# alessioGalatolo/GAN-2D-to-3D

Measured on AMD Instinct MI355X. Metric: GAN2Shape step iters/sec, faces 128×128 b=8, 1/2/4/8 MI355X, higher is better.
Workload: dtype f32; 1 GPU; face128_n8; image_size=128, gan_size=128, n_proj_samples=8, mfma_operands=f32, prior=ellipsoid, step_mix=7:7:6 (step1:step2:step3, main.py:148 stage 0), images_per_rank=1

## Files before the change

### gan-2d-to-3d_amd/csrc/modconv.hip

```cpp
#include "modconv_desc.h"
#include "conv_wgrad_core.h"
#include "thinconv.h"
#include "xcd_tile.h"

namespace g2s {

template <int T> struct KTile {
    static constexpr int BKT = (T == 9) ? 18 : (T == 25) ? 26 : 16;
    static constexpr int CPT = BKT / T;
    static constexpr int KMAX = (T == 25) ? 26 : 18;
};

template <int BM, int BN, int T, bool PARTIAL, bool SCALE>
__device__ __forceinline__ void modconv_body(const ConvDesc &d, const ConvClass &c,
                                             float (&As)[2][KTile<T>::KMAX][BM + 1],
                                             float (&Bs)[2][KTile<T>::KMAX + 1][BN],
                                             const int (&stab)[25], const int tile_id, const int grp,
                                             const int kt_begin, const int kt_end, const bool atomic) {
    constexpr int BKT = KTile<T>::BKT, CPT = KTile<T>::CPT, BK_MAX = KTile<T>::KMAX;
    constexpr int WAVES_M = BM >= 64 ? 2 : 1, WAVES_N = 4 / WAVES_M;
    constexpr int WMT = BM / (32 * WAVES_M), WNT = BN / (32 * WAVES_N);
    constexpr bool WIDE = (T == 9);
    constexpr int EA = WIDE ? (BM * 6 + NTHREADS - 1) / NTHREADS : (BM * BKT + NTHREADS - 1) / NTHREADS;
    constexpr int EB = (BN * BKT + NTHREADS - 1) / NTHREADS;
    const int tid = threadIdx.x, lane = tid & 63, wave = tid >> 6;
    const int wm = wave / WAVES_N, wn = wave % WAVES_N;
    const int Ncls = d.B * c.OH * c.OW;
    const int tiles_m = (d.M + BM - 1) / BM;
    const int m0 = (tile_id % tiles_m) * BM;
    const int n0 = (tile_id / tiles_m) * BN;
    const int HW = d.H * d.W;
    constexpr int OOB = 0x7fffffff;

    const auto rx = __builtin_amdgcn_make_buffer_rsrc((void *)(d.x + (size_t)grp * d.Cr * HW), 0,
                                                      (d.B * d.Cx - grp * d.Cr) * HW * 4, 0x00020000);
    const auto rw = __builtin_amdgcn_make_buffer_rsrc((void *)(d.w + (size_t)grp * (d.w_bytes / 4)), 0, d.w_bytes, 0x00020000);
    const auto rsc = __builtin_amdgcn_make_buffer_rsrc(
        (void *)(SCALE ? d.in_scale : d.w), 0, SCALE ? d.B * d.Cr * 4 : 4, 0x00020000);

    const int nB = tid % BN;
    const int ng = n0 + nB;
    const bool n_ok = ng < Ncls;
    int bb = 0, iy0 = 0, ix0 = 0;
    if (n_ok) {
        bb = ng / (c.OH * c.OW);
        const int r = ng % (c.OH * c.OW);
        iy0 = (r / c.OW) * d.is;
        ix0 = (r % c.OW) * d.is;
    }
    int offB[EB], dchB[EB];
#pragma unroll
// ... 121 lines not shown
                for (int j = 0; j < WNT; j++) {
                    acc[i][j] = __builtin_amdgcn_mfma_f32_32x32x2f32(a[p][i], b[p][j], acc[i][j], 0, 0, 0);
                    if (slot == 0 && st < EA) storeA(st, anext);
                    if (slot == (WMT * WNT > 1 ? 1 : 0) && st < EA) loadA(st, kt2);
                    if (slot == (WMT * WNT > 2 ? 2 : 0) && st < EB) storeB(st, bnext);
                    if (slot == (WMT * WNT > 3 ? 3 : 0) && st < EB) loadB(st, kt2);
                    slot++;
                }
            __builtin_amdgcn_sched_group_barrier(0x100, WMT + WNT, 0);
            for (int q = 0; q < WMT * WNT; q++) {
                __builtin_amdgcn_sched_group_barrier(0x008, 1, 0);
                __builtin_amdgcn_sched_group_barrier(0x200, 1, 0);
                __builtin_amdgcn_sched_group_barrier(0x020, 2, 0);
                __builtin_amdgcn_sched_group_barrier(0x002, 4, 0);
            }
        }
        if constexpr (WIDE && SCALE) { rs[0] = rsn[0]; rs[1] = rsn[1]; }
        asm volatile("s_waitcnt lgkmcnt(0)\n\ts_barrier" ::: "memory");
    };
    int kt = kt_begin;
    for (; kt + 1 < kt_end; kt += 2) {
        ktile(kt, 0);
        ktile(kt + 1, 1);
    }
    if (kt < kt_end) ktile(kt, 0);

#pragma unroll
    for (int j = 0; j < WNT; j++) {
        const int n = n0 + wn * (BN / WAVES_N) + j * 32 + l31;
        if (n >= Ncls) continue;
        const int b = n / (c.OH * c.OW);
        const int r_ = n % (c.OH * c.OW);
        const int oy = (r_ / c.OW) * d.os + c.oy0, ox = (r_ % c.OW) * d.os + c.ox0;
        float *yb = d.y + (((size_t)b * d.My + grp * d.M) * d.OHf + oy) * d.OWf + ox;
        const float *ob = d.out_scale ? d.out_scale + (size_t)b * d.M : nullptr;
        const float *gbias = d.bias ? d.bias + grp * d.M : nullptr;
        const float nz = d.noise ? d.noise_w[0] * d.noise[oy * d.OWf + ox] : 0.0f;
#pragma unroll
        for (int i = 0; i < WMT; i++)
#pragma unroll
            for (int r = 0; r < 16; r++) {
                const int m = m0 + wm * (BM / WAVES_M) + i * 32 + (r & 3) + 8 * (r >> 2) + 4 * lk;
                if (m >= d.M) continue;
                float v = acc[i][j][r];
                if (ob) v *= ob[m];
                if (gbias) v += gbias[m];
                v += nz;
                if (d.act) v = (v > 0.0f ? v : v * d.act_alpha) * d.act_gain;
                float *dst = yb + (size_t)m * d.OHf * d.OWf;
                if (atomic) unsafeAtomicAdd(dst, v);
                else *dst = v;
            }
    }
}

static __host__ __device__ inline int ktiles_of(int Cr, int T) {
    const int cpt = (T == 9) ? 2 : (T == 25) ? 1 : 16 / T;
    return (Cr + cpt - 1) / cpt;
}

template <int BM, int BN, int KMAX>
__device__ __forceinline__ void modconv_segment(const ConvDesc &d, const ConvClass &c,
                                                float (&As)[2][KMAX][BM + 1], float (&Bs)[2][KMAX + 1][BN],
                                                const int (&stab)[25], const int tile_id, const int grp,
                                                const int kb, const int ke, const bool atomic) {
    const bool scale = d.in_scale != nullptr;
#define G2S_BODY(T, PART, SC) modconv_body<BM, BN, T, PART, SC>(d, c, As, Bs, stab, tile_id, grp, kb, ke, atomic)
#define G2S_TAPS(T, CPT)                                   \
    if (d.Cr % CPT) {                                      \
        if (scale) G2S_BODY(T, true, true);                \
        else G2S_BODY(T, true, false);                     \
    } else {                                               \
        if (scale) G2S_BODY(T, false, true);               \
        else G2S_BODY(T, false, false);                    \
    }
    if constexpr (KMAX == 26) {
        G2S_BODY(25, true, false);
    } else {
        switch (c.T) {
        case 9: G2S_TAPS(9, 2) break;
        case 16: G2S_BODY(16, true, false); break;
        case 4: G2S_TAPS(4, 4) break;
        case 2: G2S_TAPS(2, 8) break;
        default: G2S_TAPS(1, 16) break;
        }
    }
#undef G2S_TAPS
#undef G2S_BODY
}

template <int BM, int BN, int KMAX>
__device__ __forceinline__ void modconv_block(const ConvDesc &d, float (&As)[2][KMAX][BM + 1],
                                              float (&Bs)[2][KMAX + 1][BN], int (&stab)[25], const int nx,
                                              const int bx, const int by, const int bz, const int row) {
    const int tiles_m = (d.M + BM - 1) / BM;
    const int tile_all0 = __builtin_amdgcn_readfirstlane(xcd_logical_tile(nx, bx, row));
    const ConvClass &c = d.cls[bz];
    const int mt_all = tile_all0 % (tiles_m * d.groups);
    const int grp = __builtin_amdgcn_readfirstlane(mt_all / tiles_m);
    const int tile_id = __builtin_amdgcn_readfirstlane((tile_all0 / (tiles_m * d.groups)) * tiles_m + mt_all % tiles_m);
    if ((int)(tile_id / tiles_m) * BN >= d.B * c.OH * c.OW) return;
    const int ktiles = ktiles_of(d.Cr, c.T);
    const int slices = d.cls_splitk[bz];
    const int per = (ktiles + slices - 1) / slices;
    const int kb = by * per;
    if (by >= slices || kb >= ktiles) return;
    if (threadIdx.x < 25) stab[threadIdx.x] = c.tab[threadIdx.x];
    __syncthreads();
    modconv_segment<BM, BN, KMAX>(d, c, As, Bs, stab, tile_id, grp, kb, min(ktiles, kb + per), slices > 1);
}

template <int BM, int BN, int KMAX>
__global__ __launch_bounds__(NTHREADS) void modconv_kernel(ConvDesc d) {
    __shared__ float As[2][KMAX][BM + 1];
    __shared__ float Bs[2][KMAX + 1][BN];
    __shared__ int stab[25];
    modconv_block<BM, BN, KMAX>(d, As, Bs, stab, gridDim.x, blockIdx.x, blockIdx.y, blockIdx.z,
                                blockIdx.y + gridDim.y * blockIdx.z);
}

__global__ __launch_bounds__(NTHREADS) void conv_wgrad_rider_kernel(WgradParams p) {
    __shared__ float Wa[WG_BK][WG_BM + 1];
    __shared__ float Wb[WG_BK][WG_BN + 1];
    wgrad_block(p, Wa, Wb, blockIdx.x, blockIdx.y, blockIdx.z);
}

template <int BM, int BN, int KMAX>
__global__ __launch_bounds__(NTHREADS) void conv_bwd_kernel(ConvDesc d, WgradParams p, int nx, int ny, int n_dgrad,
                                                            int w_tiles, int w_split) {
    __shared__ float As[2][KMAX][BM + 1];
    __shared__ float Bs[2][KMAX + 1][BN];
    __shared__ int stab[25];
    __shared__ float Wa[WG_BK][WG_BM + 1];
    __shared__ float Wb[WG_BK][WG_BN + 1];
    const int lin = blockIdx.x;
    if (lin < n_dgrad) {
        const int bx = lin % nx, row = lin / nx;
        modconv_block<BM, BN, KMAX>(d, As, Bs, stab, nx, bx, row % ny, row / ny, row);
    } else {
        const int l = lin - n_dgrad;
        const int bx = l % w_tiles, r = l / w_tiles;
        wgrad_block(p, Wa, Wb, bx, r % w_split, r / w_split);
    }
}

}

using namespace g2s;

struct TunedConv { int B, Cin, Cout, H, k, mode, transpose, fused, tile, splitk; };
static const TunedConv kTuned[] = {
#include "modconv_tuned.inc"
    {0, 0, 0, 0, 0, 0, 0, 0, 0, 0}};
// ... 21 lines not shown

struct WgradRider {
    WgradParams p;
    int tiles, split;
    bool dw_is_zero;
};

struct Epilogue {
    const float *bias, *noise, *noise_w;
    int act;
    float alpha, gain;
};

template <int KMAX>
static void conv_launch_tile(const ConvDesc &d, const dim3 grid, const int pick, hipStream_t st,
                             const WgradRider *rider = nullptr) {
    const int n_dgrad = grid.x * grid.y * grid.z;
#define G2S_TILE(BM_, BN_)                                                                                           \
    if (rider)                                                                                                       \
        conv_bwd_kernel<BM_, BN_, KMAX><<<n_dgrad + rider->tiles * rider->split * rider->p.groups, NTHREADS, 0, st>>>( \
            d, rider->p, grid.x, grid.y, n_dgrad, rider->tiles, rider->split);                                       \
    else                                                                                                             \
        modconv_kernel<BM_, BN_, KMAX><<<grid, NTHREADS, 0, st>>>(d)
    switch (pick) {
    case 0: modconv_kernel<128, 128, KMAX><<<grid, NTHREADS, 0, st>>>(d); break;
    case 1: modconv_kernel<128, 64, KMAX><<<grid, NTHREADS, 0, st>>>(d); break;
    case 2: G2S_TILE(64, 64); break;
    case 3: G2S_TILE(32, 128); break;
    default: G2S_TILE(64, 128); break;
    }
#undef G2S_TILE
}

static int conv_launch(const float *x, const float *w, const float *in_scale, const float *out_scale,
                       const Epilogue &ep, float *y, int B, int Cr, int M, int H, int W, const ConvGeom &g,
                       int tuned_tile, int tuned_splitk, g2s_stream_t stream, bool y_is_zero = false,
                       bool f16_operands = false, int groups = 1, const WgradRider *rider = nullptr,
                       int *plan_needs_zero = nullptr) {
    G2S_REQUIRE(plan_needs_zero || (x && w && y), "x, w, y must not be NULL");
    G2S_REQUIRE(B > 0 && Cr > 0 && M > 0 && H > 0 && W > 0, "sizes must be positive");
    const int k = g.k, s_ = g.stride, p_ = g.pad, KK = k * k;
    G2S_REQUIRE(k >= 1 && k <= 5, "kernel size must be 1..5 (got %d)", k);
    G2S_REQUIRE(s_ == 1 || s_ == 2, "stride must be 1 or 2 (got %d)", s_);
    G2S_REQUIRE(p_ >= 0 && p_ < k, "padding must be in [0, k)");
    ConvDesc d{};
    d.x = x;
    d.w = w;
    d.in_scale = in_scale;
    d.out_scale = out_scale;
    d.bias = ep.bias;
    d.noise = ep.noise;
    d.noise_w = ep.noise_w;
    G2S_REQUIRE(!d.noise || (!f16_operands && groups == 1), "the noise epilogue exists for the fp32 kernel only");
    d.act = ep.act;
    d.act_alpha = ep.alpha;
    d.act_gain = ep.gain;
    d.y = y;
    d.B = B;
    d.H = H;
    d.W = W;
    d.Cr = Cr;
    d.M = M;
    d.w_ms = g.m_major ? Cr * KK : KK;
    d.w_ks = g.m_major ? KK : M * KK;
    d.w_bytes = M * Cr * KK * 4;
    G2S_REQUIRE(groups >= 1 && groups <= 8 && (groups == 1 || (!in_scale && !out_scale && !f16_operands)),
                "grouped launches take no input / output scales and fp32 operands");
    d.groups = groups;
    d.Cx = groups * Cr;
    d.My = groups * M;
    bool holes = false;
    if (!g.adjoint) {
// ... 26 lines not shown
                c.ox0 = rx;
                c.OH = (d.OHf - ry + s_ - 1) / s_;
                c.OW = (d.OWf - rx + s_ - 1) / s_;
                c.T = 0;
                for (int ky = 0; ky < k; ky++)
                    for (int kx = 0; kx < k; kx++)
                        if ((ry + p_ - ky) % s_ == 0 && (rx + p_ - kx) % s_ == 0)
                            c.tab[c.T++] = pack((ry + p_ - ky) / s_, (rx + p_ - kx) / s_, ky * k + kx);
                if (c.T == 0 || c.OH <= 0 || c.OW <= 0) {
                    holes = holes || (c.OH > 0 && c.OW > 0);
                    continue;
                }
                d.cls[d.ncls++] = c;
            }
        G2S_REQUIRE(d.ncls > 0, "empty convolution");
    }
    bool big = false;
    for (int i = 0; i < d.ncls; i++) {
        const int T = d.cls[i].T;
        G2S_REQUIRE(T == 1 || T == 2 || T == 4 || T == 9 || T == 16 || T == 25,
                    "unsupported tap count %d (k=%d stride=%d)", T, k, s_);
        G2S_REQUIRE(!(in_scale && T > 9), "input scales are limited to kernels of up to 3x3");
        big = big || T == 25;
    }
    long nmax = 0;
    int kt_min = 1 << 30;
    for (int i = 0; i < d.ncls; i++) {
        nmax = std::max(nmax, (long)B * d.cls[i].OH * d.cls[i].OW);
        kt_min = std::min(kt_min, ktiles_of(d.Cr, d.cls[i].T));
    }
    G2S_REQUIRE(nmax < (1l << 30) && (long)B * d.Cx * H * W < (1l << 29) && (long)groups * M * Cr * KK < (1l << 29),
                "problem too large for 32-bit byte offsets");
    hipStream_t st = as_stream(stream);
    const int cfgs[5][2] = {{128, 128}, {128, 64}, {64, 64}, {32, 128}, {64, 128}};
    int pick = 2;
    for (int i = 0; i < 3; i++) {
        const long blocks = (long)groups * cdiv(d.M, cfgs[i][0]) * cdiv(nmax, cfgs[i][1]) * d.ncls;
        if (d.M > cfgs[i][0] / 2 && blocks >= 512) { pick = i; break; }
    }
    if (d.M <= 32 && nmax >= 1024 && !f16_operands) pick = 3;
    if (f16_operands && pick == 1) pick = 2;
    if (tuned_tile >= 0 && g_force_tile != -2) pick = tuned_tile;
    else tuned_splitk = -1;
    if (g_force_tile >= 0) pick = g_force_tile;
    const int BMv = cfgs[pick][0], BNv = cfgs[pick][1];
    const int tiles = groups * cdiv(d.M, BMv) * cdiv(nmax, BNv);
    int splitk = 1;
    while ((long)tiles * d.ncls * splitk < 512 && kt_min / (splitk * 2) >= 8 && splitk < 64) splitk *= 2;
    if (tuned_splitk > 0) splitk = tuned_splitk;
    if (g_force_splitk > 0) splitk = g_force_splitk;
    if (deterministic()) splitk = 1;
    splitk = std::max(1, std::min(splitk, kt_min));
    dim3 grid(tiles, splitk, d.ncls);
    const bool split = splitk > 1;
    const bool deferred_epilogue = (split || holes) && (ep.bias != nullptr || ep.act != 0 || ep.noise != nullptr);
    if (deferred_epilogue) {
        d.bias = nullptr;
        d.noise = d.noise_w = nullptr;
        d.act = 0;
    }
    d.splitk = splitk;
    int kt_max = 1;
    for (int i = 0; i < d.ncls; i++) kt_max = std::max(kt_max, ktiles_of(d.Cr, d.cls[i].T));
    for (int i = 0; i < d.ncls; i++) {
        const int kt = ktiles_of(d.Cr, d.cls[i].T);
        d.cls_splitk[i] = std::max(1, std::min(kt, (int)(((long)splitk * kt + kt_max / 2) / kt_max)));
// ... 7 lines not shown
            return fail(G2S_ERR_LAUNCH, "hipMemsetAsync(y) failed");
    }
    if (f16_operands) {
        const int rc = modconv_f16_launch(d, grid, pick, st);
        if (rc != G2S_OK) return rc;
    } else if (rider) {
        const WgradParams &p = rider->p;
        if (p.atomic && !rider->dw_is_zero &&
            hipMemsetAsync(p.dw, 0, (size_t)p.groups * p.Ca * p.N * sizeof(float), st) != hipSuccess)
            return fail(G2S_ERR_LAUNCH, "hipMemsetAsync(dw) failed");
        if (big) conv_launch_tile<26>(d, grid, pick, st, pick >= 2 ? rider : nullptr);
        else conv_launch_tile<18>(d, grid, pick, st, pick >= 2 ? rider : nullptr);
        if (pick < 2) conv_wgrad_rider_kernel<<<dim3(rider->tiles, rider->split, p.groups), NTHREADS, 0, st>>>(p);
    } else if (big) {
        conv_launch_tile<26>(d, grid, pick, st);
    } else {
        conv_launch_tile<18>(d, grid, pick, st);
    }
    int rc = check_launch("g2s_modconv");
    if (rc != G2S_OK || !deferred_epilogue) return rc;
    if (ep.noise) {
        G2S_REQUIRE(ep.bias && ep.act == 1, "noise epilogue: needs a bias and act = 1");
        return g2s_noise_bias_act(y, ep.noise, ep.noise_w, ep.bias, y, B, d.My, d.OHf * d.OWf, ep.alpha, ep.gain,
                                  stream);
    }
    return g2s_fused_bias_act(y, ep.bias, nullptr, y, (int64_t)B * d.My * d.OHf * d.OWf,
                              (int64_t)d.OHf * d.OWf, d.My, ep.act ? 3 : 1, 0, ep.alpha,
                              ep.act ? ep.gain : 1.0f, G2S_F32, stream);
}

static int modconv_launch(const float *x, const float *w, const float *in_scale,
                          const float *out_scale, const Epilogue &ep, float *y, int B, int Cin, int Cout, int H,
                          int W, int k, int mode, int transpose, g2s_stream_t stream, bool f16_operands = false,
                          bool y_is_zero = false, int *plan_needs_zero = nullptr) {
    G2S_REQUIRE(B > 0 && Cin > 0 && Cout > 0 && H > 0 && W > 0, "sizes must be positive");
    G2S_REQUIRE(k == 1 || k == 3, "kernel size must be 1 or 3 (got %d)", k);
    G2S_REQUIRE(mode == G2S_CONV_PLAIN || mode == G2S_CONV_UP2 || mode == G2S_CONV_DOWN2,
                "unsupported mode %d", mode);
    if (!f16_operands && !in_scale && !out_scale && !ep.noise && mode == G2S_CONV_PLAIN && g_force_tile == -1 &&
        g_force_splitk == -1 && thin_conv_eligible(B, Cin, Cout, H, W, k, transpose)) {
        if (plan_needs_zero) {
            *plan_needs_zero = 0;
            return G2S_OK;
        }
        return thin_conv_launch(x, w, ep.bias, y, B, Cin, Cout, H, W, ep.act, ep.alpha, ep.gain, stream);
    }
    ConvGeom g{};
    g.k = k;
    g.stride = mode == G2S_CONV_PLAIN ? 1 : 2;
    g.pad = mode == G2S_CONV_PLAIN ? k / 2 : 0;
    g.adjoint = (mode == G2S_CONV_UP2) != (transpose != 0);
    g.m_major = !transpose;
    if (!g.adjoint && mode != G2S_CONV_PLAIN) G2S_REQUIRE(H >= k && W >= k, "input smaller than the kernel");
    int tile = -1, splitk = -1;
    if (H == W && !f16_operands)
        for (int pass = 0; pass < 2 && tile == -1 && splitk == -1; pass++)
            for (const TunedConv *t = kTuned; t->B; ++t)
                if (t->B == B && t->Cin == Cin && t->Cout == Cout && t->H == H && t->k == k && t->mode == mode &&
                    t->transpose == transpose && (pass == 1 || t->fused == (ep.bias != nullptr || ep.act != 0))) {
                    tile = t->tile;
                    splitk = t->splitk;
                    break;
                }
    return conv_launch(x, w, in_scale, out_scale, ep, y, B, transpose ? Cout : Cin, transpose ? Cin : Cout, H, W, g,
                       tile, splitk, stream, y_is_zero, f16_operands, 1, nullptr, plan_needs_zero);
}

extern "C" int g2s_modconv(const float *x, const float *w, const float *in_scale, const float *out_scale,
                           const float *bias, const float *noise, const float *noise_w, float *y, int B, int Cin,
                           int Cout, int H, int W, int k, int mode, int transpose, int act, float alpha, float gain,
                           int y_is_zero, g2s_stream_t stream) {
    G2S_REQUIRE(act == 0 || act == 1, "act must be 0 (none) or 1 (leaky-ReLU)");
    G2S_REQUIRE(!noise || (bias && noise_w && act == 1), "a noise needs bias, noise_w and act = 1");
    return modconv_launch(x, w, in_scale, out_scale, Epilogue{bias, noise, noise_w, act, alpha, gain}, y, B, Cin,
                          Cout, H, W, k, mode, transpose, stream, false, y_is_zero != 0);
}

extern "C" int g2s_modconv_needs_zero(int B, int Cin, int Cout, int H, int W, int k, int mode, int transpose,
                                      int has_scales, int fused) {
    int needs = 0;
    static const float dummy = 0.0f;
    const float *sc = has_scales ? &dummy : nullptr;
    const Epilogue ep{fused ? &dummy : nullptr, nullptr, nullptr, fused ? 1 : 0, 0.0f, 1.0f};
    const int rc = modconv_launch(nullptr, nullptr, sc, nullptr, ep, nullptr, B, Cin, Cout, H, W, k, mode, transpose,
                                  nullptr, false, false, &needs);
    return rc == G2S_OK ? needs : rc;
}

extern "C" int g2s_modconv_f16(const float *x, const float *w, const float *in_scale, const float *out_scale,
                               const float *bias, float *y, int B, int Cin, int Cout, int H, int W, int k,
                               int mode, int transpose, int act, float alpha, float gain, g2s_stream_t stream) {
    G2S_REQUIRE(act == 0 || act == 1, "act must be 0 (none) or 1 (leaky-ReLU)");
    return modconv_launch(x, w, in_scale, out_scale, Epilogue{bias, nullptr, nullptr, act, alpha, gain}, y, B, Cin,
                          Cout, H, W, k, mode, transpose, stream, true);
}

static int conv2d_impl(const float *x, const float *w, const float *bias, float *y, int B, int Cr, int M, int H,
                       int W, int k, int stride, int pad, int adjoint, int w_m_major, int out_h, int out_w,
                       int act, float alpha, float gain, int y_is_zero, int groups, g2s_stream_t stream,
                       const WgradRider *rider = nullptr) {
    G2S_REQUIRE(act == 0 || act == 1, "act must be 0 (none) or 1 (leaky-ReLU)");
    ConvGeom g{k, stride, pad, adjoint ? 1 : 0, w_m_major ? 1 : 0, adjoint ? out_h : 0, adjoint ? out_w : 0};
    int tile = -1, splitk = -1;
    if (H == W)
        for (const TunedConv2d *t = kTuned2d; t->B; ++t)
            if (t->B == B && t->Cr == Cr && t->M == M && t->H == H && t->k == k && t->stride == stride &&
                t->pad == pad && t->adjoint == g.adjoint && t->m_major == g.m_major &&
                t->fused == (bias != nullptr || act != 0) && t->groups == groups) {
// ... 28 lines not shown
```

### gan-2d-to-3d_amd/lib.py

```python
import ctypes as C
import os

import torch

_HERE = os.path.dirname(os.path.abspath(__file__))
LIB_PATH = os.path.join(_HERE, "lib", "libg2s.so")

G2S_F32, G2S_F16 = 0, 1
CONV_PLAIN, CONV_UP2, CONV_DOWN2 = 0, 1, 2

_lib = None

_p, _i, _f, _sz, _i64, _d = C.c_void_p, C.c_int, C.c_float, C.c_size_t, C.c_int64, C.c_double
SIGNATURES = {
    "g2s_abi_version": (_i, []),
    "g2s_last_error": (C.c_char_p, []),
    "g2s_clamp": (_i, [_p, _p, _p, _i64, _f, _f, _i, _p]),
    "g2s_avg_pyramid": (_i, [_p, _p, _i, _i64, _i, _i, _p]),
    "g2s_res_split_fwd": (_i, [_p, _p, _p, _i64, _i, _i, _p]),
    "g2s_res_split_bwd": (_i, [_p, _p, _p, _p, _i64, _i, _i, _p]),
    "g2s_depth_head_fwd": (_i, [_p, _p, _p, _i64, _i, _f, _f, _i, _f, _p]),
    "g2s_depth_head_bwd": (_i, [_p, _p, _p, _p, _p, _i64, _i, _f, _f, _i, _f, _i, _p]),
    "g2s_grid_sample_fwd": (_i, [_p, _p, _p, _i, _i, _i, _i, _i, _i, _i, _f, _f, _p]),
    "g2s_grid_sample_bwd_workspace_bytes": (_sz, [_i, _i, _i, _i]),
# ... 1 lines not shown
    "g2s_set_deterministic": (_i, [_i]),
    "g2s_get_deterministic": (_i, []),
    "g2s_raster_workspace_bytes": (_sz, [_i, _i, _i, _i]),
    "g2s_raster_tune": (_i, [_i]),
    "g2s_raster_get_tune": (_i, []),
    "g2s_raster_depth_fwd": (_i, [_p, _p, _i, _i, _i, _i, _p, _f, _i, _i, _f, _f, _p, _p, _p, _p, _sz, _p]),
    "g2s_raster_depth_bwd": (_i, [_p, _p, _p, _p, _p, _i, _i, _i, _i, _p, _f, _i, _p, _p]),
    "g2s_raster_bwd_workspace_bytes": (_sz, [_i, _i]),
    "g2s_raster_depth_bwd_ex": (_i, [_p, _p, _p, _p, _p, _i, _i, _i, _i, _p, _f, _i, _p, _p, _sz, _i, _p]),
    "g2s_raster_rgb_fwd": (_i, [_p, _p, _p, _p, _p, _i, _i, _i, _i, _i, _i, _i, _p, _f, _p, _p]),
    "g2s_raster_rgb_bwd_workspace_bytes": (_sz, [_i, _i, _i, _i, _i]),
    "g2s_raster_rgb_bwd": (_i, [_p] * 6 + [_i, _i, _i, _i, _p, _f, _i, _i, _i, _f, _p, _p, _p, _sz, _i, _p]),
    "g2s_face_light_fwd": (_i, [_p, _p, _i, _i, _i, _i, _i, _p, _p, _p, _p, _p]),
    "g2s_face_light_bwd": (_i, [_p, _p, _p, _i, _i, _i, _i, _i, _p, _p, _p, _p, _sz, _i, _p]),
    "g2s_raster_rgba_fwd": (_i, [_p] * 6 + [_i, _i, _i, _i, _i, _i, _i, _i, _p, _f, _p, _p, _p]),
    "g2s_raster_rgba_bwd_workspace_bytes": (_sz, [_i, _i, _i, _i, _i, _i]),
    "g2s_raster_rgba_bwd": (_i, [_p] * 7 + [_i, _i, _i, _i, _p, _f, _i, _i, _i, _i, _f, _p, _p, _p, _p, _sz, _i, _p]),
    "g2s_sweep_verts": (_i, [_p, _p, _p, _i, _i, _i, _p]),
    "g2s_sweep_shade": (_i, [_p] * 8 + [_i] * 9 + [_p, _f, _p, _p, _p]),
    "g2s_sweep_pseudo": (_i, [_p] * 8 + [_f, _f, _i, _i, _i, _i, _p, _p, _p]),
    "g2s_mapping_tile": (_i, []),
    "g2s_mapping_fwd": (_i, [_p, _p, _p, _p, _p, _p, _i64, _i, _i, _i, _f, _f, _f, _p]),
    "g2s_rows_mean": (_i, [_p, _p, _i64, _i, _i64, _p]),
    "g2s_image_to_u8": (_i, [_p, _p, _i64, _i, _i, _p]),
    "g2s_fused_bias_act": (_i, [_p, _p, _p, _p, _i64, _i64, _i64, _i, _i, _f, _f, _i, _p]),
    "g2s_maxpool2x2_fwd": (_i, [_p, _p, _i64, _i, _i, _p]),
    "g2s_maxpool2x2_bwd": (_i, [_p, _p, _p, _i64, _i, _i, _p]),
    "g2s_add_bias_scale": (_i, [_p, _p, _p, _p, _i64, _i64, _i, _f, _p]),
    "g2s_noise_bias_act": (_i, [_p, _p, _p, _p, _p, _i, _i, _i, _f, _f, _p]),
    "g2s_noise_bias_act_ps": (_i, [_p, _p, _p, _p, _p, _i, _i, _i, _f, _f, _p]),
    "g2s_upfirdn2d": (_i, [_p, _p, _p] + [_i] * 14 + [_p]),
    "g2s_modconv": (_i, [_p] * 8 + [_i] * 9 + [_f, _f, _i, _p]),
    "g2s_modconv_needs_zero": (_i, [_i, _i, _i, _i, _i, _i, _i, _i, _i, _i]),
    "g2s_upfirdn2d_nba": (_i, [_p, _p, _p] + [_i] * 12 + [_p, _p, _p, _f, _f, _p]),
    "g2s_synth_bwd_rows": (_i, [_p] * 13 + [_i, _i, _i, _f, _f, _p]),
    "g2s_upfirdn2d_nba_ps": (_i, [_p, _p, _p] + [_i] * 12 + [_p, _p, _p, _f, _f, _p]),
    "g2s_synth_bwd_rows_ps": (_i, [_p] * 13 + [_i, _i, _i, _f, _f, _p]),
    "g2s_channel_sum": (_i, [_p, _p, _i, _i, _i, _p]),
    "g2s_noise_grad": (_i, [_p, _p, _p, _i, _i, _i, _p]),
    "g2s_noise_regularize_workspace_bytes": (_sz, [_p, _i, _i]),
    "g2s_noise_regularize": (_i, [_p, _p, _p, _i, _i, _p, _p, _sz, _p]),
    "g2s_noise_normalize_workspace_bytes": (_sz, [_p, _i, _i]),
    "g2s_noise_normalize": (_i, [_p, _p, _i, _i, _p, _sz, _p]),
    "g2s_demod_fwd_multi": (_i, [_p, _p, _p, _p, _p, _i, _i, _f, _p]),
    "g2s_demod_bwd_multi": (_i, [_p, _p, _p, _p, _p, _p, _p, _i, _i, _p]),
    "g2s_modconv_f16": (_i, [_p, _p, _p, _p, _p, _p, _i, _i, _i, _i, _i, _i, _i, _i, _i, _f, _f, _p]),
    "g2s_modconv_tune": (_i, [_i, _i]),
    "g2s_mfma_probe": (_i, [_p, _i, _i, _i, _p]),
    "g2s_mfma_lds_probe": (_i, [_p, _i, _i, _i, _i, _p]),
    "g2s_wino_weights_floats": (_sz, [_i, _i]),
    "g2s_wino4_weights_floats": (_sz, [_i, _i]),
    "g2s_wino4_weights": (_i, [_p, _p, _i, _i, _i, _p]),
    "g2s_wino4_supported": (_i, [_i] * 5),
    "g2s_conv3x3_wino4": (_i, [_p] * 8 + [_i] * 6 + [_f, _f, _i, _p, _i64, _p]),
    "g2s_wino_weights": (_i, [_p, _p, _i, _i, _i, _p]),
    "g2s_conv3x3_wino": (_i, [_p] * 8 + [_i] * 6 + [_f, _f, _i, _p, _i64, _p]),
    "g2s_conv2d": (_i, [_p, _p, _p, _p] + [_i] * 12 + [_i, _f, _f, _i, _i, _p]),
    "g2s_conv2d_wgrad": (_i, [_p, _p, _p] + [_i] * 10 + [_i, _i, _p]),
    "g2s_conv2d_bwd": (_i, [_p, _p, _p] + [_i] * 13 + [_p, _p, _p] + [_i] * 8 + [_p]),
    "g2s_adam_chunk": (_i64, []),
    "g2s_adam_step": (_i, [_p, _p, _p, _i, _i, _f, _f, _f, _f, _f, _p]),
    "g2s_rows_dot_scale": (_i, [_p, _p, _p, _p, _p, _p, _i, _i, _p]),
    "g2s_demod_fwd": (_i, [_p, _p, _p, _i, _i, _i, _f, _p]),
    "g2s_demod_bwd": (_i, [_p, _p, _p, _p, _p, _i, _i, _i, _p]),
    "g2s_demod_bwd_add": (_i, [_p, _p, _p, _p, _p, _p, _i, _i, _i, _p]),
    "g2s_lpips_layer_fwd": (_i, [_p, _p, _p, _p, _i, _i, _i, _p]),
# ... 124 lines not shown
```

### gan-2d-to-3d_amd/modconv.py

```python
import os

import torch
from torch.autograd import Function

from . import lib as _lib
from . import zeropool as _zp

PLAIN, UP2, DOWN2 = _lib.CONV_PLAIN, _lib.CONV_UP2, _lib.CONV_DOWN2

PROFILE = None


class profiled:

    def __init__(self, flop, nbytes, mfma_flop=None, kernel=None):
        self.rec = PROFILE
        self.flop, self.nbytes = flop, nbytes
        self.kernel = kernel or ("direct" if mfma_flop is None else "winograd")
        self.mfma_flop = flop if mfma_flop is None else mfma_flop

    def __enter__(self):
        if self.rec is not None:
            self.e0 = torch.cuda.Event(enable_timing=True)
            self.e1 = torch.cuda.Event(enable_timing=True)
# ... 51 lines not shown
    if tiles < WINO_MIN_TILES or blocks * -(-Cr // 4) < 256 * 32 or M <= 32:
        return None
    return 0


WINO4 = os.environ.get("G2S_WINO4", "1") != "0"


def wino4_supported(B, Cr, M, H, W):
    return WINO4 and _lib.load().g2s_wino4_supported(B, Cr, M, H, W) == 1


_WINO_U = {"winograd": {}, "winograd4": {}}


def _wino_weights(w, transpose, kernel):
    cache = _WINO_U[kernel]
    key = (w.data_ptr(), w._version, tuple(w.shape), int(transpose))
    hit = cache.get(key)
    if hit is None:
        if len(cache) > 256:
            cache.clear()
        Cout, Cin = w.shape[:2]
        L = _lib.load()
        M, Cr = (Cin, Cout) if transpose else (Cout, Cin)
        floats, transform = ((L.g2s_wino4_weights_floats, L.g2s_wino4_weights) if kernel == "winograd4"
                             else (L.g2s_wino_weights_floats, L.g2s_wino_weights))
        U = torch.empty(floats(M, Cr), dtype=torch.float32, device=w.device)
        _lib.check(transform(_lib.ptr(w), _lib.ptr(U), Cout, Cin, int(transpose), _lib.stream()))
        hit = cache[key] = (w, U)
    return hit[1]


def _conv(x, w, in_scale, out_scale, mode, transpose, out_shape, route, bias=None, noise=None, noise_w=None, act=0,
          alpha=0.0, gain=1.0):
    B, Cr, H, W = x.shape
    Cout, Cin, k, _ = w.shape
    M = out_shape[1]
    act, alpha, gain = int(act), float(alpha), float(gain)
    L = _lib.load()
    p = _lib.ptr
    y = None
    if route is None and L.g2s_modconv_needs_zero(B, Cin, Cout, H, W, k, mode, int(transpose),
                                                  int(in_scale is not None or out_scale is not None),
                                                  int(bias is not None or act != 0)) == 1:
        y = _zp.take(out_shape, x.device)
    zeroed = y is not None
    if y is None:
        y = torch.empty(out_shape, dtype=torch.float32, device=x.device)
    oh, ow = out_shape[2], out_shape[3]
    flop = 2.0 * B * Cout * Cin * k * k * (oh * ow if mode == PLAIN else min(H * W, oh * ow))
    nbytes = 4.0 * (x.numel() + w.numel() + y.numel())
    if route is None:
        with profiled(flop, nbytes):
            _lib.check(L.g2s_modconv(p(x), p(w), p(in_scale), p(out_scale), p(bias), p(noise), p(noise_w), p(y), B,
                                     Cin, Cout, H, W, k, mode, int(transpose), act, alpha, gain, int(zeroed),
                                     _lib.stream()))
    elif route == "f16":
        with profiled(flop, nbytes):
            _lib.check(L.g2s_modconv_f16(p(x), p(w), p(in_scale), p(out_scale), p(bias), p(y), B, Cin, Cout, H, W, k,
                                         mode, int(transpose), act, alpha, gain, _lib.stream()))
    elif isinstance(route, str):
        U = _wino_weights(w, transpose, "winograd4")
        with profiled(flop, nbytes, 2.0 * 36 * B * (H // 4) * (W // 4) * M * Cr, "winograd4"):
            _lib.check(L.g2s_conv3x3_wino4(p(x), p(U), p(in_scale), p(out_scale), p(bias), p(noise), p(noise_w), p(y),
                                           B, Cr, M, H, W, act, alpha, gain, int(route[3:] or 0), *_lib.split_ws(),
                                           _lib.stream()))
    else:
        U = _wino_weights(w, transpose, "winograd")
        tiles = B * ((H + 1) // 2) * ((W + 1) // 2)
        with profiled(flop, nbytes, 2.0 * 16 * tiles * M * Cr):
            _lib.check(L.g2s_conv3x3_wino(p(x), p(U), p(in_scale), p(out_scale), p(bias), p(noise), p(noise_w), p(y),
                                          B, Cr, M, H, W, act, alpha, gain, int(route), *_lib.split_ws(),
                                          _lib.stream()))
    return y


def modconv_nba_raw(x, w, in_scale, out_scale, bias, noise, noise_w, slope, gain):
    _lib.require_cuda(x, w, in_scale, out_scale, bias, noise, noise_w)
    if OPERANDS != "f32" or x.dtype != torch.float32:
        raise RuntimeError("modconv_nba: fp32 kernels only")
    x, w = x.contiguous(), w.contiguous()
    B, C, H, W = x.shape
    Cout, Cin = w.shape[:2]
    if C != Cin or tuple(noise.shape[-2:]) != (H, W) or noise.numel() != H * W:
        raise RuntimeError("modconv_nba: shape mismatch")
    si, so = in_scale.contiguous(), out_scale.contiguous()
    bias, noise, noise_w = bias.contiguous(), noise.contiguous(), noise_w.contiguous()
    return _conv(x, w, si, so, PLAIN, 0, (B, Cout, H, W), wino_choice(x, w, PLAIN, 0, 1), bias, noise, noise_w, 1,
                 slope, gain)


def modconv_raw(x, w, in_scale, out_scale, mode, transpose):
    _lib.require_cuda(x, w, in_scale, out_scale)
# ... 241 lines not shown
```

### include/g2s.h

```cpp
#ifndef G2S_H
#define G2S_H

#include <stddef.h>
#include <stdint.h>

#ifdef __cplusplus
extern "C" {
#endif

#define G2S_ABI_VERSION 1

#define G2S_OK 0
#define G2S_ERR_INVALID (-1)
#define G2S_ERR_LAUNCH (-2)
#define G2S_ERR_WORKSPACE (-3)

#define G2S_F32 0
#define G2S_F16 1

typedef void *g2s_stream_t;

int g2s_abi_version(void);
const char *g2s_last_error(void);

// ... 110 lines not shown
                        int IH, int IW, int H, int W, int clamp, float lo, float hi, void *workspace,
                        size_t workspace_bytes, int acc_is_zero, g2s_stream_t stream);

int g2s_clamp(const float *x, const float *g, float *y, int64_t n, float lo, float hi, int backward,
              g2s_stream_t stream);

int g2s_noise_bias_act(const float *x, const float *noise, const float *noise_w,
                       const float *bias, float *y, int B, int C, int HW, float alpha,
                       float scale, g2s_stream_t stream);
int g2s_noise_bias_act_ps(const float *x, const float *noise, const float *noise_w, const float *bias, float *y, int B,
                          int C, int HW, float alpha, float scale, g2s_stream_t stream);

int g2s_upfirdn2d(const void *x, const float *k, void *y, int major, int in_h, int in_w, int kh,
                  int kw, int up_x, int up_y, int down_x, int down_y, int pad_x0, int pad_x1,
                  int pad_y0, int pad_y1, int dtype, g2s_stream_t stream);
int g2s_upfirdn2d_nba(const float *x, const float *k, float *y, int major, int channels, int in_h, int in_w, int kh,
                      int kw, int up, int down, int pad_x0, int pad_x1, int pad_y0, int pad_y1, const float *bias,
                      const float *noise, const float *noise_w, float alpha, float gain, g2s_stream_t stream);
int g2s_upfirdn2d_nba_ps(const float *x, const float *k, float *y, int major, int channels, int in_h, int in_w, int kh,
                         int kw, int up, int down, int pad_x0, int pad_x1, int pad_y0, int pad_y1, const float *bias,
                         const float *noise, const float *noise_w, float alpha, float gain, g2s_stream_t stream);



#define G2S_CONV_PLAIN 0
#define G2S_CONV_UP2 1
#define G2S_CONV_DOWN2 2

int g2s_modconv(const float *x, const float *w, const float *in_scale, const float *out_scale, const float *bias,
                const float *noise, const float *noise_w, float *y, int B, int Cin, int Cout, int H, int W, int k,
                int mode, int transpose, int act, float alpha, float gain, int y_is_zero, g2s_stream_t stream);
int g2s_modconv_needs_zero(int B, int Cin, int Cout, int H, int W, int k, int mode, int transpose,
                           int has_scales, int fused);

int g2s_conv2d(const float *x, const float *w, const float *bias, float *y, int B, int Cr, int M, int H,
               int W, int k, int stride, int pad, int adjoint, int w_m_major, int out_h, int out_w,
               int act, float alpha, float gain, int y_is_zero, int groups, g2s_stream_t stream);
int g2s_conv2d_wgrad(const float *A, const float *G, float *dw, int B, int Ca, int Cg, int PH, int PW,
                     int GH, int GW, int k, int stride, int pad, int dw_is_zero, int groups, g2s_stream_t stream);

int g2s_conv2d_bwd(const float *gy, const float *w, float *gx, int B, int Cr, int M, int H, int W, int k,
                   int stride, int pad, int adjoint, int w_m_major, int out_h, int out_w, int gx_is_zero,
                   const float *A, const float *G, float *dw, int Ca, int Cg, int PH, int PW, int GH, int GW,
                   int dw_is_zero, int groups, g2s_stream_t stream);

#define G2S_ADAM_MAX_TENSORS 128
typedef struct g2s_adam_tensor {
    float *p, *m, *v;
    int64_t n;
    float *step;
    int *ticket;
} g2s_adam_tensor;
int64_t g2s_adam_chunk(void);
int g2s_adam_step(const g2s_adam_tensor *tensors, const int *chunk0, const float *const *grads, int n_tensors,
                  int n_chunks, float lr, float beta1, float beta2, float eps, float weight_decay,
                  g2s_stream_t stream);

int g2s_modconv_f16(const float *x, const float *w, const float *in_scale, const float *out_scale,
                    const float *bias, float *y, int B, int Cin, int Cout, int H, int W, int k, int mode,
                    int transpose, int act, float alpha, float gain, g2s_stream_t stream);

size_t g2s_wino_weights_floats(int M, int Cr);
int g2s_wino_weights(const float *w, float *U, int Cout, int Cin, int transpose, g2s_stream_t stream);
int g2s_conv3x3_wino(const float *x, const float *U, const float *in_scale, const float *out_scale,
                     const float *bias, const float *noise, const float *noise_w, float *y, int B, int Cr, int M,
                     int H, int W, int act, float alpha, float gain, int splitk, float *ws, int64_t ws_floats,
// ... 196 lines not shown
```

Before: 206.1 iters/s.

## Add equal-length split-K unit launch for stride-2 modulated convs with separate reduce

Adds a stride-2 modconv path that splits every phase class's K range into roughly equal-length work units. All units run in one flat grid and write partial results to a workspace, then a second kernel sums the slices and applies bias, noise and activation. The aim is to balance work across phase classes with different tap counts and fill the CUs for small-spatial 512-channel layers, in place of atomic split-K with uneven slices. It costs an extra reduce kernel launch and workspace traffic. A tuned table enables it only for the 4x4 and 8x8 512-channel up2 shapes.

```diff
diff --git a/gan-2d-to-3d_amd/csrc/modconv.hip b/gan-2d-to-3d_amd/csrc/modconv.hip
--- a/gan-2d-to-3d_amd/csrc/modconv.hip
+++ b/gan-2d-to-3d_amd/csrc/modconv.hip
@@ -1,4 +1,6 @@
 #include "modconv_desc.h"
+#include "modconv_units.h"
+#include "split_reduce.h"
 #include "conv_wgrad_core.h"
 #include "thinconv.h"
 #include "xcd_tile.h"
@@ -16,7 +18,8 @@
                                              float (&As)[2][KTile<T>::KMAX][BM + 1],
                                              float (&Bs)[2][KTile<T>::KMAX + 1][BN],
                                              const int (&stab)[25], const int tile_id, const int grp,
-                                             const int kt_begin, const int kt_end, const bool atomic) {
+                                             const int kt_begin, const int kt_end, const bool atomic,
+                                             float *const part = nullptr) {
     constexpr int BKT = KTile<T>::BKT, CPT = KTile<T>::CPT, BK_MAX = KTile<T>::KMAX;
     constexpr int WAVES_M = BM >= 64 ? 2 : 1, WAVES_N = 4 / WAVES_M;
     constexpr int WMT = BM / (32 * WAVES_M), WNT = BN / (32 * WAVES_N);
@@ -204,7 +207,9 @@
         const int b = n / (c.OH * c.OW);
         const int r_ = n % (c.OH * c.OW);
         const int oy = (r_ / c.OW) * d.os + c.oy0, ox = (r_ % c.OW) * d.os + c.ox0;
-        float *yb = d.y + (((size_t)b * d.My + grp * d.M) * d.OHf + oy) * d.OWf + ox;
+        const size_t plane = part ? (size_t)c.OH * c.OW : (size_t)d.OHf * d.OWf;
+        float *yb = part ? part + (size_t)b * d.M * plane + r_
+                         : d.y + (((size_t)b * d.My + grp * d.M) * d.OHf + oy) * d.OWf + ox;
         const float *ob = d.out_scale ? d.out_scale + (size_t)b * d.M : nullptr;
         const float *gbias = d.bias ? d.bias + grp * d.M : nullptr;
         const float nz = d.noise ? d.noise_w[0] * d.noise[oy * d.OWf + ox] : 0.0f;
@@ -219,7 +224,7 @@
                 if (gbias) v += gbias[m];
                 v += nz;
                 if (d.act) v = (v > 0.0f ? v : v * d.act_alpha) * d.act_gain;
-                float *dst = yb + (size_t)m * d.OHf * d.OWf;
+                float *dst = yb + (size_t)m * plane;
                 if (atomic) unsafeAtomicAdd(dst, v);
                 else *dst = v;
             }
@@ -235,9 +240,10 @@
 __device__ __forceinline__ void modconv_segment(const ConvDesc &d, const ConvClass &c,
                                                 float (&As)[2][KMAX][BM + 1], float (&Bs)[2][KMAX + 1][BN],
                                                 const int (&stab)[25], const int tile_id, const int grp,
-                                                const int kb, const int ke, const bool atomic) {
+                                                const int kb, const int ke, const bool atomic,
+                                                float *const part = nullptr) {
     const bool scale = d.in_scale != nullptr;
-#define G2S_BODY(T, PART, SC) modconv_body<BM, BN, T, PART, SC>(d, c, As, Bs, stab, tile_id, grp, kb, ke, atomic)
+#define G2S_BODY(T, PART, SC) modconv_body<BM, BN, T, PART, SC>(d, c, As, Bs, stab, tile_id, grp, kb, ke, atomic, part)
 #define G2S_TAPS(T, CPT)                                   \
     if (d.Cr % CPT) {                                      \
         if (scale) G2S_BODY(T, true, true);                \
@@ -291,6 +297,73 @@
                                 blockIdx.y + gridDim.y * blockIdx.z);
 }
 
+template <int BM, int BN>
+__global__ __launch_bounds__(NTHREADS) void modconv_units_kernel(ConvDesc d, UnitPlan p, float *ws) {
+    __shared__ float As[2][18][BM + 1];
+    __shared__ float Bs[2][19][BN];
+    __shared__ int stab[25];
+    const int u = __builtin_amdgcn_readfirstlane(xcd_logical_tile(gridDim.x, blockIdx.x, 0));
+    if (u >= p.total) return;
+    int ci = 0;
+    for (int i = 1; i < UNITS_MAX_CLASSES; i++)
+        if (i < p.ncls && u >= p.cls[i].first) ci = i;
+    ci = __builtin_amdgcn_readfirstlane(ci);
+    const UnitClass &uc = p.cls[ci];
+    const ConvClass &c = d.cls[ci];
+    const int local = u - uc.first;
+    const int slice = __builtin_amdgcn_readfirstlane(local / uc.tiles);
+    const int tile_id = __builtin_amdgcn_readfirstlane(local - slice * uc.tiles);
+    int kb, ke;
+    unit_krange(uc, slice, kb, ke);
+    if (threadIdx.x < 25) stab[threadIdx.x] = c.tab[threadIdx.x];
+    __syncthreads();
+    modconv_segment<BM, BN, 18>(d, c, As, Bs, stab, tile_id, 0, __builtin_amdgcn_readfirstlane(kb),
+                                __builtin_amdgcn_readfirstlane(ke), false, ws + uc.ws_off + (size_t)slice * uc.n);
+}
+
+struct UnitsReduce {
+    float *y;
+    const float *bias, *noise, *noise_w;
+    int M, OHf, OWf, os, act;
+    float alpha, gain;
+    int64_t n;
+    int cmap[4];
+};
+
+__global__ __launch_bounds__(256) void modconv_units_reduce_kernel(UnitPlan p, UnitsReduce r, const float *ws) {
+    const float nw = r.noise ? r.noise_w[0] : 0.0f;
+    const int64_t stride = (int64_t)gridDim.x * blockDim.x;
+    for (int64_t i = (int64_t)blockIdx.x * blockDim.x + threadIdx.x; i < r.n; i += stride) {
+        const int ox = (int)(i % r.OWf);
+        const int64_t t = i / r.OWf;
+        const int oy = (int)(t % r.OHf);
+        const int64_t bm = t / r.OHf;
+        const int ry = oy % r.os, rx = ox % r.os;
+        int ci = -1;
+#pragma unroll
+        for (int k = 0; k < 4; k++)
+            if (k == ry * r.os + rx) ci = r.cmap[k];
+        float v = 0.0f;
+#pragma unroll
+        for (int k = 0; k < UNITS_MAX_CLASSES; k++)
+            if (k == ci) {
+                const UnitClass &uc = p.cls[k];
+                const float *src = ws + uc.ws_off + (bm * uc.OH + oy / r.os) * uc.OW + ox / r.os;
+                float part[UNITS_MAX_SLICES];
+#pragma unroll
+                for (int s = 0; s < UNITS_MAX_SLICES; s++)
+                    if (s < uc.slices) part[s] = src[(int64_t)s * uc.n];
+#pragma unroll
+                for (int s = 0; s < UNITS_MAX_SLICES; s++)
+                    if (s < uc.slices) v += part[s];
+            }
+        if (r.bias) v += r.bias[bm % r.M];
+        if (r.noise) v += nw * r.noise[oy * r.OWf + ox];
+        if (r.act) v = (v > 0.0f ? v : v * r.alpha) * r.gain;
+        r.y[i] = v;
+    }
+}
+
 __global__ __launch_bounds__(NTHREADS) void conv_wgrad_rider_kernel(WgradParams p) {
     __shared__ float Wa[WG_BK][WG_BM + 1];
     __shared__ float Wb[WG_BK][WG_BN + 1];
@@ -378,12 +451,70 @@
 #undef G2S_TILE
 }
 
+struct UnitsReq {
+    int len;
+    float *ws;
+    int64_t ws_floats;
+    int64_t *plan_floats;
+};
+
+static int units_launch(ConvDesc &d, const Epilogue &ep, const UnitsReq &u, hipStream_t st, g2s_stream_t stream) {
+    for (int i = 1; i < d.ncls; i++)
+        for (int j = i; j > 0 && d.cls[j].T > d.cls[j - 1].T; j--) std::swap(d.cls[j], d.cls[j - 1]);
+    const bool wide = d.M <= 32;
+    const int BMv = wide ? 32 : 64, BNv = wide ? 128 : 64;
+    int kt[4], tiles[4], OH[4], OW[4];
+    UnitsReduce r{};
+    for (int k = 0; k < 4; k++) r.cmap[k] = -1;
+    for (int i = 0; i < d.ncls; i++) {
+        const ConvClass &c = d.cls[i];
+        G2S_REQUIRE(c.T <= 9, "unit launches serve kernels of up to 3x3");
+        kt[i] = ktiles_of(d.Cr, c.T);
+        tiles[i] = cdiv(d.M, BMv) * cdiv(d.B * c.OH * c.OW, BNv);
+        OH[i] = c.OH;
+        OW[i] = c.OW;
+        r.cmap[c.oy0 * d.os + c.ox0] = i;
+    }
+    UnitPlan p{};
+    G2S_REQUIRE(units_plan(kt, tiles, OH, OW, d.ncls, (int64_t)d.B * d.M, u.len, 256, p),
+                "no equal-length unit partition for this launch");
+    if (u.plan_floats) {
+        *u.plan_floats = p.ws_floats;
+        return G2S_OK;
+    }
+    G2S_REQUIRE(u.ws && u.ws_floats >= p.ws_floats, "workspace too small: %lld floats given, %lld needed",
+                (long long)u.ws_floats, (long long)p.ws_floats);
+    d.bias = nullptr;
+    d.noise = d.noise_w = nullptr;
+    d.act = 0;
+    d.splitk = 1;
+    if (wide) modconv_units_kernel<32, 128><<<p.total, NTHREADS, 0, st>>>(d, p, u.ws);
+    else modconv_units_kernel<64, 64><<<p.total, NTHREADS, 0, st>>>(d, p, u.ws);
+    const int rc = check_launch("g2s_modconv_units");
+    if (rc != G2S_OK) return rc;
+    r.y = d.y;
+    r.bias = ep.bias;
+    r.noise = ep.noise;
+    r.noise_w = ep.noise_w;
+    r.M = d.M;
+    r.OHf = d.OHf;
+    r.OWf = d.OWf;
+    r.os = d.os;
+    r.act = ep.act;
+    r.alpha = ep.alpha;
+    r.gain = ep.gain;
+    r.n = (int64_t)d.B * d.M * d.OHf * d.OWf;
+    const int blocks = (int)std::min<int64_t>((r.n + 255) / 256, 256 * 8);
+    modconv_units_reduce_kernel<<<blocks, 256, 0, st>>>(p, r, u.ws);
+    return check_launch("g2s_modconv_units reduce");
+}
+
 static int conv_launch(const float *x, const float *w, const float *in_scale, const float *out_scale,
                        const Epilogue &ep, float *y, int B, int Cr, int M, int H, int W, const ConvGeom &g,
                        int tuned_tile, int tuned_splitk, g2s_stream_t stream, bool y_is_zero = false,
                        bool f16_operands = false, int groups = 1, const WgradRider *rider = nullptr,
-                       int *plan_needs_zero = nullptr) {
-    G2S_REQUIRE(plan_needs_zero || (x && w && y), "x, w, y must not be NULL");
+                       int *plan_needs_zero = nullptr, const UnitsReq *units = nullptr) {
+    G2S_REQUIRE(plan_needs_zero || (units && units->plan_floats) || (x && w && y), "x, w, y must not be NULL");
     G2S_REQUIRE(B > 0 && Cr > 0 && M > 0 && H > 0 && W > 0, "sizes must be positive");
     const int k = g.k, s_ = g.stride, p_ = g.pad, KK = k * k;
     G2S_REQUIRE(k >= 1 && k <= 5, "kernel size must be 1..5 (got %d)", k);
@@ -476,6 +607,12 @@
     G2S_REQUIRE(nmax < (1l << 30) && (long)B * d.Cx * H * W < (1l << 29) && (long)groups * M * Cr * KK < (1l << 29),
                 "problem too large for 32-bit byte offsets");
     hipStream_t st = as_stream(stream);
+    if (units) {
+        G2S_REQUIRE(!big && !f16_operands && groups == 1 && !rider && !plan_needs_zero && s_ == 2,
+                    "unit launches: stride-2 fp32 launches of one group");
+        G2S_REQUIRE(!ep.noise || (ep.bias && ep.act == 1), "noise epilogue: needs a bias and act = 1");
+        return units_launch(d, ep, *units, st, stream);
+    }
     const int cfgs[5][2] = {{128, 128}, {128, 64}, {64, 64}, {32, 128}, {64, 128}};
     int pick = 2;
     for (int i = 0; i < 3; i++) {
@@ -549,7 +686,7 @@
 static int modconv_launch(const float *x, const float *w, const float *in_scale,
                           const float *out_scale, const Epilogue &ep, float *y, int B, int Cin, int Cout, int H,
                           int W, int k, int mode, int transpose, g2s_stream_t stream, bool f16_operands = false,
-                          bool y_is_zero = false, int *plan_needs_zero = nullptr) {
+                          bool y_is_zero = false, int *plan_needs_zero = nullptr, const UnitsReq *units = nullptr) {
     G2S_REQUIRE(B > 0 && Cin > 0 && Cout > 0 && H > 0 && W > 0, "sizes must be positive");
     G2S_REQUIRE(k == 1 || k == 3, "kernel size must be 1 or 3 (got %d)", k);
     G2S_REQUIRE(mode == G2S_CONV_PLAIN || mode == G2S_CONV_UP2 || mode == G2S_CONV_DOWN2,
@@ -570,7 +707,7 @@
     g.m_major = !transpose;
     if (!g.adjoint && mode != G2S_CONV_PLAIN) G2S_REQUIRE(H >= k && W >= k, "input smaller than the kernel");
     int tile = -1, splitk = -1;
-    if (H == W && !f16_operands)
+    if (H == W && !f16_operands && !units)
         for (int pass = 0; pass < 2 && tile == -1 && splitk == -1; pass++)
             for (const TunedConv *t = kTuned; t->B; ++t)
                 if (t->B == B && t->Cin == Cin && t->Cout == Cout && t->H == H && t->k == k && t->mode == mode &&
@@ -580,7 +717,7 @@
                     break;
                 }
     return conv_launch(x, w, in_scale, out_scale, ep, y, B, transpose ? Cout : Cin, transpose ? Cin : Cout, H, W, g,
-                       tile, splitk, stream, y_is_zero, f16_operands, 1, nullptr, plan_needs_zero);
+                       tile, splitk, stream, y_is_zero, f16_operands, 1, nullptr, plan_needs_zero, units);
 }
 
 extern "C" int g2s_modconv(const float *x, const float *w, const float *in_scale, const float *out_scale,
@@ -591,6 +728,30 @@
     G2S_REQUIRE(!noise || (bias && noise_w && act == 1), "a noise needs bias, noise_w and act = 1");
     return modconv_launch(x, w, in_scale, out_scale, Epilogue{bias, noise, noise_w, act, alpha, gain}, y, B, Cin,
                           Cout, H, W, k, mode, transpose, stream, false, y_is_zero != 0);
+}
+
+extern "C" int g2s_modconv_units(const float *x, const float *w, const float *in_scale, const float *out_scale,
+                                 const float *bias, const float *noise, const float *noise_w, float *y, int B,
+                                 int Cin, int Cout, int H, int W, int k, int mode, int transpose, int act,
+                                 float alpha, float gain, int unit_ktiles, float *ws, int64_t ws_floats,
+                                 g2s_stream_t stream) {
+    G2S_REQUIRE(act == 0 || act == 1, "act must be 0 (none) or 1 (leaky-ReLU)");
+    G2S_REQUIRE(!noise || (bias && noise_w && act == 1), "a noise needs bias, noise_w and act = 1");
+    G2S_REQUIRE(mode == G2S_CONV_UP2 || mode == G2S_CONV_DOWN2, "unit launches serve the stride-2 modes");
+    G2S_REQUIRE(unit_ktiles >= 0, "unit_ktiles must be >= 0");
+    const UnitsReq u{unit_ktiles, ws, ws_floats, nullptr};
+    return modconv_launch(x, w, in_scale, out_scale, Epilogue{bias, noise, noise_w, act, alpha, gain}, y, B, Cin,
+                          Cout, H, W, k, mode, transpose, stream, false, false, nullptr, &u);
+}
+
+extern "C" int64_t g2s_modconv_units_ws_floats(int B, int Cin, int Cout, int H, int W, int k, int mode, int transpose,
+                                               int unit_ktiles) {
+    int64_t floats = 0;
+    const UnitsReq u{unit_ktiles, nullptr, 0, &floats};
+    if (unit_ktiles < 0 || (mode != G2S_CONV_UP2 && mode != G2S_CONV_DOWN2)) return -1;
+    const int rc = modconv_launch(nullptr, nullptr, nullptr, nullptr, Epilogue{nullptr, nullptr, nullptr, 0, 0.0f, 1.0f},
+                                  nullptr, B, Cin, Cout, H, W, k, mode, transpose, nullptr, false, false, nullptr, &u);
+    return rc == G2S_OK ? floats : -1;
 }
 
 extern "C" int g2s_modconv_needs_zero(int B, int Cin, int Cout, int H, int W, int k, int mode, int transpose,
diff --git a/gan-2d-to-3d_amd/csrc/modconv_units.h b/gan-2d-to-3d_amd/csrc/modconv_units.h
--- /dev/null
+++ b/gan-2d-to-3d_amd/csrc/modconv_units.h
@@ -0,0 +1,99 @@
+#pragma once
+#include <cstdint>
+
+#ifdef __HIPCC__
+#define G2S_UNITS_HD __host__ __device__
+#else
+#define G2S_UNITS_HD
+#endif
+
+namespace g2s {
+
+constexpr int UNITS_MAX_SLICES = 8;
+constexpr int UNITS_MAX_CLASSES = 4;
+
+struct UnitClass {
+    int first;
+    int tiles;
+    int slices;
+    int ktiles;
+    int OH, OW;
+    int64_t n;
+    int64_t ws_off;
+};
+
+struct UnitPlan {
+    int ncls;
+    int total;
+    int len;
+    int64_t ws_floats;
+    UnitClass cls[UNITS_MAX_CLASSES];
+};
+
+static G2S_UNITS_HD inline void unit_krange(const UnitClass &c, int s, int &kb, int &ke) {
+    const int base = c.ktiles / c.slices, rem = c.ktiles % c.slices;
+    kb = s * base + (s < rem ? s : rem);
+    ke = kb + base + (s < rem ? 1 : 0);
+}
+
+static inline bool units_feasible(const int *ktiles, int ncls, int len, int *slices) {
+    if (len < 1) return false;
+    for (int i = 0; i < ncls; i++) {
+        const int s = (ktiles[i] + len) / (len + 1);
+        if (s < 1 || s > UNITS_MAX_SLICES || s * len > ktiles[i]) return false;
+        slices[i] = s;
+    }
+    return true;
+}
+
+constexpr int UNIT_FIXED = 6;
+
+static inline bool units_plan(const int *ktiles, const int *tiles, const int *OH, const int *OW, int ncls,
+                              int64_t BM, int want_len, int cus, UnitPlan &p) {
+    if (ncls < 1 || ncls > UNITS_MAX_CLASSES || cus < 1) return false;
+    int kt_min = ktiles[0], kt_max = ktiles[0];
+    for (int i = 1; i < ncls; i++) {
+        kt_min = ktiles[i] < kt_min ? ktiles[i] : kt_min;
+        kt_max = ktiles[i] > kt_max ? ktiles[i] : kt_max;
+    }
+    if (kt_min < 1) return false;
+    int slices[UNITS_MAX_CLASSES], best = 0;
+    if (want_len > 0) {
+        for (int len = want_len < kt_min ? want_len : kt_min; len >= 1 && !best; len--)
+            if (units_feasible(ktiles, ncls, len, slices)) best = len;
+        for (int len = want_len + 1; len <= kt_min && !best; len++)
+            if (units_feasible(ktiles, ncls, len, slices)) best = len;
+    } else {
+        int64_t best_cost = 0;
+        for (int len = 1; len <= kt_min; len++) {
+            if (!units_feasible(ktiles, ncls, len, slices)) continue;
+            int64_t units = 0;
+            for (int i = 0; i < ncls; i++) units += (int64_t)tiles[i] * slices[i];
+            const int64_t cost = ((units + cus - 1) / cus) * (len + 1 + UNIT_FIXED);
+            if (!best || cost < best_cost) { best = len; best_cost = cost; }
+        }
+    }
+    if (!best || !units_feasible(ktiles, ncls, best, slices)) return false;
+    p.ncls = ncls;
+    p.len = best;
+    int64_t off = 0, total = 0;
+    for (int i = 0; i < ncls; i++) {
+        UnitClass &c = p.cls[i];
+        c.first = (int)total;
+        c.tiles = tiles[i];
+        c.slices = slices[i];
+        c.ktiles = ktiles[i];
+        c.OH = OH[i];
+        c.OW = OW[i];
+        c.n = BM * OH[i] * OW[i];
+        c.ws_off = off;
+        off += c.n * slices[i];
+        total += (int64_t)tiles[i] * slices[i];
+    }
+    if (total > (1 << 24)) return false;
+    p.total = (int)total;
+    p.ws_floats = off;
+    return true;
+}
+
+}
diff --git a/gan-2d-to-3d_amd/lib.py b/gan-2d-to-3d_amd/lib.py
--- a/gan-2d-to-3d_amd/lib.py
+++ b/gan-2d-to-3d_amd/lib.py
@@ -57,6 +57,8 @@
     "g2s_upfirdn2d": (_i, [_p, _p, _p] + [_i] * 14 + [_p]),
     "g2s_modconv": (_i, [_p] * 8 + [_i] * 9 + [_f, _f, _i, _p]),
     "g2s_modconv_needs_zero": (_i, [_i, _i, _i, _i, _i, _i, _i, _i, _i, _i]),
+    "g2s_modconv_units": (_i, [_p] * 8 + [_i] * 9 + [_f, _f, _i, _p, _i64, _p]),
+    "g2s_modconv_units_ws_floats": (_i64, [_i] * 9),
     "g2s_upfirdn2d_nba": (_i, [_p, _p, _p] + [_i] * 12 + [_p, _p, _p, _f, _f, _p]),
     "g2s_synth_bwd_rows": (_i, [_p] * 13 + [_i, _i, _i, _f, _f, _p]),
     "g2s_upfirdn2d_nba_ps": (_i, [_p, _p, _p] + [_i] * 12 + [_p, _p, _p, _f, _f, _p]),
diff --git a/gan-2d-to-3d_amd/modconv.py b/gan-2d-to-3d_amd/modconv.py
--- a/gan-2d-to-3d_amd/modconv.py
+++ b/gan-2d-to-3d_amd/modconv.py
@@ -107,6 +107,23 @@
     return hit[1]
 
 
+try:
+    from .units_tuned import TABLE as _UNITS_TABLE
+except ImportError:
+    _UNITS_TABLE = {}
+UNITS_FORCE = None
+
+
+def units_choice(x, w, mode, transpose):
+    if mode == PLAIN or w.shape[2] != 3 or UNITS_FORCE == "off":
+        return None
+    if UNITS_FORCE is not None:
+        return f"u:{int(UNITS_FORCE)}"
+    B, _, H, W = x.shape
+    hit = _UNITS_TABLE.get((B, w.shape[1], w.shape[0], H, W, int(mode), int(transpose)))
+    return None if hit is None else f"u:{int(hit)}"
+
+
 def _conv(x, w, in_scale, out_scale, mode, transpose, out_shape, route, bias=None, noise=None, noise_w=None, act=0,
           alpha=0.0, gain=1.0):
     B, Cr, H, W = x.shape
@@ -116,6 +133,8 @@
     L = _lib.load()
     p = _lib.ptr
     y = None
+    if route is None and mode != PLAIN and OPERANDS == "f32":
+        route = units_choice(x, w, mode, transpose)
     if route is None and L.g2s_modconv_needs_zero(B, Cin, Cout, H, W, k, mode, int(transpose),
                                                   int(in_scale is not None or out_scale is not None),
                                                   int(bias is not None or act != 0)) == 1:
@@ -135,6 +154,11 @@
         with profiled(flop, nbytes):
             _lib.check(L.g2s_modconv_f16(p(x), p(w), p(in_scale), p(out_scale), p(bias), p(y), B, Cin, Cout, H, W, k,
                                          mode, int(transpose), act, alpha, gain, _lib.stream()))
+    elif isinstance(route, str) and route.startswith("u:"):
+        with profiled(flop, nbytes):
+            _lib.check(L.g2s_modconv_units(p(x), p(w), p(in_scale), p(out_scale), p(bias), p(noise), p(noise_w), p(y),
+                                           B, Cin, Cout, H, W, k, mode, int(transpose), act, alpha, gain,
+                                           int(route[2:]), *_lib.split_ws(), _lib.stream()))
     elif isinstance(route, str):
         U = _wino_weights(w, transpose, "winograd4")
         with profiled(flop, nbytes, 2.0 * 36 * B * (H // 4) * (W // 4) * M * Cr, "winograd4"):
diff --git a/gan-2d-to-3d_amd/units_tuned.py b/gan-2d-to-3d_amd/units_tuned.py
--- /dev/null
+++ b/gan-2d-to-3d_amd/units_tuned.py
@@ -0,0 +1,4 @@
+TABLE = {
+    (8, 512, 512, 4, 4, 1, 0): 16,
+    (8, 512, 512, 8, 8, 1, 0): 32,
+}
diff --git a/include/g2s.h b/include/g2s.h
--- a/include/g2s.h
+++ b/include/g2s.h
@@ -166,6 +166,13 @@
                 int mode, int transpose, int act, float alpha, float gain, int y_is_zero, g2s_stream_t stream);
 int g2s_modconv_needs_zero(int B, int Cin, int Cout, int H, int W, int k, int mode, int transpose,
                            int has_scales, int fused);
+
+int g2s_modconv_units(const float *x, const float *w, const float *in_scale, const float *out_scale,
+                      const float *bias, const float *noise, const float *noise_w, float *y, int B, int Cin, int Cout,
+                      int H, int W, int k, int mode, int transpose, int act, float alpha, float gain, int unit_ktiles,
+                      float *ws, int64_t ws_floats, g2s_stream_t stream);
+int64_t g2s_modconv_units_ws_floats(int B, int Cin, int Cout, int H, int W, int k, int mode, int transpose,
+                                    int unit_ktiles);
 
 int g2s_conv2d(const float *x, const float *w, const float *bias, float *y, int B, int Cr, int M, int H,
                int W, int k, int stride, int pad, int adjoint, int w_m_major, int out_h, int out_w,
```

Result: no change. 204.5 iters/s (-0.8%).
